# DavidSevic/gpu-nbody-simulation

Hardware: AMD Instinct MI355X
Metric: body-steps/sec (higher is better)
Workload: dtype f32

## Files before the change

### gpu-nbody-simulation_amd/csrc/bh_engine.hip

```cpp
#include "../../include/bhgpu.h"

#include <hip/hip_runtime.h>

#include <algorithm>
#include <cmath>
#include <cstdio>
#include <cstdlib>
#include <cstring>
#include <string>
#include <type_traits>
#include <vector>

#include "bh_tree.hpp"
#include "bh_walk_exact.hpp"
#include "bh_walk_f64.hpp"
#include "bh_diag.hpp"
#include "bh_direct.hpp"
#include "bh_field.hpp"
#include "bh_init.hpp"
#include "bh_let.hpp"
#include "bh_migrate.hpp"
#include "bh_walk_fast.h"

using namespace bh;
// ... 8 lines not shown
};
#endif

namespace {

thread_local std::string g_create_error;

struct DevBuf {
    void *p = nullptr;
    size_t bytes = 0;
};

}

struct bh_ctx {
    bh_config cfg{};
    int Dm = 0;
    enum class Mode { Exact, F64, Mixed, F32 };
    Mode mode = Mode::Exact;
    bool tree64() const { return mode == Mode::Exact || mode == Mode::F64; }
    bool state64() const { return mode != Mode::F32; }
    bool compat = true;
    bool exact_thresholds = false;
    int device = 0;
    hipStream_t stream = nullptr;
    bool own_stream = false;
    int64_t n = 0;
    bool uploaded = false, tree_valid = false;
    int64_t internal_cap = 0, node_cap = 0;
    int64_t bfs_max = 12288;
    int exact_bpw = 0;
    int walk_split = 0;
    bool walk_asm = true;
    int sort_bucket = 1;
    bool last_sort_bucket = false, last_sort_packed = false;
    int64_t samples_n = -1;
    uint64_t *splitters = nullptr;
    uint16_t *sort_dig = nullptr;
    int build_items = 0;
    bool hilbert = false;
    int partial_count = 0;
    double *bslots = nullptr;
    bool slots_valid = false;
    bool slots_dirty = true;

    void *pos = nullptr, *vel = nullptr, *mass = nullptr, *force = nullptr;
    void *pos2 = nullptr, *vel2 = nullptr, *mass2 = nullptr, *force2 = nullptr;
    uint32_t *orig = nullptr, *orig2 = nullptr;
    bool orig_identity = true;
    int reorder_every = 16;
    int64_t builds = 0;
    float2 *spos = nullptr;
    float4 *sstate = nullptr;
    float *smass = nullptr;
    uint64_t *keys[2] = {nullptr, nullptr};
    uint32_t *vals[2] = {nullptr, nullptr};
    uint64_t *keys_sorted = nullptr;
    uint32_t *perm = nullptr;
    uint32_t *radix_counts = nullptr, *bsum_sort = nullptr, *bsum_u32 = nullptr, *cnt = nullptr;
    uint64_t *coarse = nullptr;
    uint32_t *cell_first = nullptr;
    d3 *terms = nullptr, *bsum_d3 = nullptr;
    double *partial = nullptr, *box = nullptr;
    NodeD *gd = nullptr;
    LinkD *ld = nullptr;
    QuadF *qf = nullptr;
// ... 459 lines not shown
                               c->cfg.dt, w.integrate ? 1 : 0, c->ctr, w.slots, k.bpw, c->box);
        };
        dispatch([&](auto compat) {
            constexpr bool CP = decltype(compat)::value;
            if (!c->exact_thresholds) { if (w.stats) go(walk_exact_kernel<CP, true, false, false>); else go(walk_exact_kernel<CP, false, false, false>); }
            else if (w.stats) go(walk_exact_kernel<CP, true, true, false>);
            else if (k.use_asm) go(walk_exact_kernel<CP, false, true, true>);
            else go(walk_exact_kernel<CP, false, true, false>);
        }, c->compat);
        return BH_OK;
    });
}

int launch_walk_f32(bh_ctx *c, const WalkRange &w, const WalkChoice &k)
{
    WalkFastArgs a{};
    a.quads = c->qf; a.aux = c->aux; a.partial = w.partial; a.spos = c->spos; a.smass = c->smass; a.perm = c->perm;
    a.pos = (float2 *)c->pos; a.vel = (float2 *)c->vel;
    a.state64 = c->state64() ? 1 : 0;
    a.sstate = c->sstate;
    a.acc_out = (float2 *)c->force; a.ctr = c->ctr;
    a.lo = w.lo; a.hi = w.hi; a.G = (float)c->cfg.G; a.dt = (float)c->cfg.dt;
    a.integrate = w.integrate ? 1 : 0; a.to_sorted = w.to_sorted ? 1 : 0;
    a.n_trees = c->let_mode ? c->world : 0; a.self_rank = c->let_mode ? c->rank : -1;
    a.part = w.part; a.acc_part = c->acc_part;
    a.forest_base = c->forest_base; a.let_cap = c->let_cap;
    c->exp.walk_args(a);
    a.group_cost = (w.lo == 0 && w.hi == c->n) ? c->group_cost : nullptr;
    a.bucket_consts = c->walk_consts;
    a.slots = w.slots;
    a.body_counts = w.stats ? c->body_counts : nullptr;
    const bool lds = (c->cfg.flags & BH_FLAG_LDS_STACK) != 0;
    a.pair_limit = std::max(0, 116 - 3 * c->Dm);
    int split = (c->cfg.flags & BH_FLAG_WALK_NO_SPLIT) || c->cfg.n_threads > 0 ? 1 : c->walk_split;
    if (split <= 0) {
        const int64_t groups = (w.hi - w.lo + kWave - 1) / kWave;
        split = groups <= (c->let_mode ? 512 : 768) ? 8 : groups <= 3072 ? 4 : 1;
    }
    if (3 * c->Dm + 2 > kWave) split = 1;
    const int per_record = walk_fast_split_effective(a, lds, split) ? kWave : kBlock;
    if (w.partial) c->partial_count = (int)blocks_for(w.hi - w.lo, per_record);
    return each_pass(c, w, per_record, [&](int64_t plo, int64_t phi, unsigned) -> int {
        a.lo = plo; a.hi = phi; a.partial = w.partial ? w.partial + 4 * ((plo - w.lo) / per_record) : nullptr;
        BH_HIP(c, launch_walk_fast(a, lds, w.stats, split, k.use_asm, c->stream));
        return BH_OK;
    });
}

int enqueue_walk(bh_ctx *c, bool integrate, bool to_sorted, int part = 0)
{
    WalkRange w{};
    owned_range(c, &w.lo, &w.hi);
    if (w.hi <= w.lo) return BH_OK;
    w.integrate = integrate; w.to_sorted = to_sorted; w.part = part;
    w.stats = (c->cfg.flags & BH_FLAG_WALK_STATS) != 0;
    if (part != 2) c->walk_launches = 0;
    w.pass = c->cfg.n_threads > 0 ? ((int64_t)c->cfg.n_threads + kBlock - 1) / kBlock * kBlock : w.hi - w.lo;
    const bool full = integrate && !to_sorted && w.lo == 0 && w.hi == c->n;
    if (full && c->let_mode) w.partial = c->partial;
    const bool want_slots = full && part == 0 && !c->let_mode && !c->external_box && c->n >= 2;
    if (want_slots) { clean_slots(c); w.slots = c->bslots; }
    if (integrate) { c->slots_valid = want_slots; c->phi_current = false; }

    const WalkChoice k = choose_walk(c, w);
    if (w.stats && (k.kind == WalkKind::F64 || k.kind == WalkKind::F32)) {
        if (!c->body_counts) { int rc = dev_alloc(c, &c->body_counts, (size_t)std::max<int64_t>(c->cfg.capacity, 1)); if (rc) return rc; }
// ... 57 lines not shown
const char *bh_build_info(void) { return BHGPU_BUILD_INFO; }

const char *bh_last_error(const bh_ctx *ctx) { return ctx ? ctx->err.c_str() : g_create_error.c_str(); }

int bh_create(const bh_config *cfg, bh_ctx **out)
{
    if (!cfg || !out) return fail(nullptr, BH_ERR_ARG, "bh_create: null argument");
    *out = nullptr;
    if (cfg->capacity < 0 || cfg->capacity > 0x7fffffffLL - 8)
        return fail(nullptr, BH_ERR_ARG, "bh_create: capacity out of range");
    if (cfg->max_depth < 1 || cfg->max_depth > 32)
        return fail(nullptr, BH_ERR_ARG, "bh_create: max_depth must be 1..32");
    if (!(cfg->theta > 0.0)) return fail(nullptr, BH_ERR_ARG, "bh_create: theta must be > 0");
    if (cfg->precision != BH_PRECISION_F64_EXACT && cfg->precision != BH_PRECISION_F32 &&
        cfg->precision != BH_PRECISION_MIXED && cfg->precision != BH_PRECISION_F64)
        return fail(nullptr, BH_ERR_ARG, "bh_create: unknown precision");
    int ndev = 0;
    if (hipGetDeviceCount(&ndev) != hipSuccess || ndev <= 0)
        return fail(nullptr, BH_ERR_NO_DEVICE, "bh_create: no HIP device (libbhgpu has no CPU fallback)");
    if (cfg->device < 0 || cfg->device >= ndev)
        return fail(nullptr, BH_ERR_ARG, "bh_create: device ordinal out of range");

    bh_ctx *c = new bh_ctx();
    c->cfg = *cfg;
    c->Dm = cfg->max_depth - 1;
    c->mode = cfg->precision == BH_PRECISION_F64_EXACT ? Mode::Exact
            : cfg->precision == BH_PRECISION_F64       ? Mode::F64
            : cfg->precision == BH_PRECISION_MIXED     ? Mode::Mixed : Mode::F32;
    c->compat = cfg->reference_compat != 0;
    c->device = cfg->device;
    if (const char *e = std::getenv("BH_WALK_SPLIT")) c->walk_split = std::atoi(e);
    if (const char *e = std::getenv("BH_EXACT_BPW")) { const int b = std::atoi(e); c->exact_bpw = (b >= 1 && b <= kWave && (b & (b - 1)) == 0) ? b : 0; }
    if (const char *e = std::getenv("BH_WALK_ASM")) c->walk_asm = std::atoi(e) != 0;
    if (const char *e = std::getenv("BH_EXACT_BFS_MAX")) c->bfs_max = std::max(0, std::atoi(e));
    c->exact_thresholds = c->mode == Mode::Exact && c->walk_asm && !(cfg->flags & BH_FLAG_WALK_PORTABLE);
    if (const char *e = std::getenv("BH_SORT_PACK")) c->sort_pack = std::atoi(e) != 0;
    if (const char *e = std::getenv("BH_SORT_BUCKET")) c->sort_bucket = std::atoi(e);
    if (const char *e = std::getenv("BH_BUILD_ITEMS")) c->build_items = std::atoi(e);
    if (const char *e = std::getenv("BH_REORDER_EVERY")) c->reorder_every = std::max(0, std::atoi(e));
    c->hilbert = !c->tree64();
    if (const char *e = std::getenv("BH_HILBERT")) c->hilbert = !c->tree64() && std::atoi(e) != 0;
    auto bail = [&](int rc) { g_create_error = c->err; bh_destroy(c); return rc; };

    if (hipSetDevice(c->device) != hipSuccess) { c->err = "hipSetDevice failed"; return bail(BH_ERR_DEVICE); }
    if (hipStreamCreateWithFlags(&c->stream, hipStreamNonBlocking) != hipSuccess) {
        c->err = "hipStreamCreate failed"; return bail(BH_ERR_DEVICE);
    }
    c->own_stream = true;

    const int64_t cap = std::max<int64_t>(cfg->capacity, 1);
    c->node_cap = cfg->node_capacity > 0 ? cfg->node_capacity : 8 * cap + 1024;
    if (c->Dm < 15) {
        int64_t full = 0, wdt = 1;
        for (int l = 0; l <= c->Dm; ++l) { full += wdt; wdt *= 4; }
        c->node_cap = std::min(c->node_cap, std::max<int64_t>(full, 1));
    }
    c->internal_cap = (c->node_cap - 1) / 4;

    const size_t rs = c->state64() ? sizeof(double) : sizeof(float);
    int rc = 0;
    auto A = [&](auto **pp, size_t count) { if (!rc) rc = dev_alloc(c, pp, count); };
    { char *t; A(&t, cap * 2 * rs); c->pos = t; }
    { char *t; A(&t, cap * 2 * rs); c->vel = t; }
    { char *t; A(&t, cap * rs); c->mass = t; }
    { char *t; A(&t, cap * 2 * (c->tree64() ? sizeof(double) : sizeof(float))); c->force = t; }
    if (!c->tree64()) {
// ... 1217 lines not shown
```

### gpu-nbody-simulation_amd/csrc/bh_walk_fast.h

```cpp
#pragma once

#include <hip/hip_runtime.h>
#include <stdint.h>

namespace bh {

struct QuadF;
struct NodeAux;
struct TreeCounters;

struct WalkFastArgs {
    const QuadF *quads;
    const NodeAux *aux;
    const float2 *spos;
    const float *smass;
    const uint32_t *perm;
    float2 *pos, *vel;
    int32_t state64;
    float4 *sstate;
    float2 *acc_out;
    TreeCounters *ctr;
    double *partial;
    int64_t lo, hi;
    float G, dt;
    int integrate, to_sorted;
    uint32_t nblocks, pad0;
    const void *bucket_consts;
    uint32_t *group_cost;
    int32_t pair_limit;
    uint64_t *timeline;
    int32_t n_trees, self_rank;
    int32_t part;
    float2 *acc_part;
    int64_t forest_base, let_cap;
    double *slots;
    uint32_t *body_counts;
};

hipError_t launch_walk_fast(const WalkFastArgs &a, bool lds_stack, bool stats, int split, bool use_asm, hipStream_t st);
inline bool walk_fast_split_effective(const WalkFastArgs &a, bool lds_stack, int split)
{
    return split > 1 && !lds_stack && a.n_trees <= 56;
}

}
```

### gpu-nbody-simulation_amd/csrc/bh_walk_fast.hip

```cpp
#include "bh_prims.hpp"
#include "bh_nodes.hpp"
#include "bh_bounds.hpp"
#include "bh_walk_fast.h"
#include <cstdlib>

namespace bh {

#define BH_CONSTANT __attribute__((address_space(4)))

extern "C" __device__ int bh_writelane_i32(int value, int lane, int old) __asm("llvm.amdgcn.writelane.i32");

template <typename T>
__device__ __forceinline__ const T BH_CONSTANT *as_constant(const T *p)
{
#pragma clang diagnostic push
#pragma clang diagnostic ignored "-Wold-style-cast"
    return (const T BH_CONSTANT *)p;
#pragma clang diagnostic pop
}

typedef int32_t v16i __attribute__((ext_vector_type(16)));
typedef int32_t v4i __attribute__((ext_vector_type(4)));
typedef int32_t v2i __attribute__((ext_vector_type(2)));
struct QuadRegs { v16i g; v4i c; };
// ... 15 lines not shown
#define BH_LOOP_GUARD ""
#endif
#define BH_FORCE_MATH(MS, MASK)                                                                     \
    "v_mul_f32_e32 v26, " MS ", v25\n"                                                              \
    "v_mul_f32_e32 v26, v25, v26\n"                                                                 \
    "v_mul_f32_e32 v24, v25, v26\n"                                                                 \
    "v_fmac_f32_e32 v28, v24, v22\n"                                                                \
    "v_fmac_f32_e32 v29, v24, v23\n"                                                                \
    "s_mov_b64 exec, " MASK "\n"
#define BH_CHILD_HEAD(XY, MS, TS, MASK, SPAIR, TAG)                                                 \
    "s_cmp_eq_u32 " MS ", 0\n"                                                                      \
    "s_cbranch_scc1 Lnext" TAG "_%=\n"                                                              \
    "v_pk_add_f32 v[22:23], " XY ", v[20:21] neg_lo:[0,1] neg_hi:[0,1]\n"                           \
    "s_nop 0\n"                                                                                     \
    "v_mul_f32_e32 v24, v23, v23\n"                                                                 \
    "v_fmac_f32_e32 v24, v22, v22\n"                                                                \
    "v_cmpx_lt_f32_e32 vcc, " TS ", v24\n"                                                          \
    "v_rsq_f32_e32 v25, v24\n"                                                                      \
    "s_andn2_b64 " SPAIR ", " MASK ", vcc\n"                                                        \
    "s_cbranch_scc0 Lforce" TAG "_%=\n"
#define BH_CHILD_T(XY, MS, TS, CS, MASK, SPAIR, SLO, SHI, TAG, PUSHCHK)                             \
    BH_CHILD_HEAD(XY, MS, TS, MASK, SPAIR, TAG)                                                     \
    "s_cmp_eq_u32 " CS ", -1\n"                                                                     \
    "s_cbranch_scc1 Lforce" TAG "_%=\n"                                                             \
    PUSHCHK                                                                                         \
    "v_writelane_b32 v30, " CS ", m0\n"                                                             \
    "v_writelane_b32 v31, " SLO ", m0\n"                                                            \
    "v_writelane_b32 v32, " SHI ", m0\n"                                                            \
    "LpushBack" TAG "_%=:\n"                                                                        \
    "s_add_u32 m0, m0, 1\n"                                                                         \
    "Lforce" TAG "_%=:\n"                                                                           \
    BH_FORCE_MATH(MS, MASK)                                                                         \
    "Lnext" TAG "_%=:\n"
#define BH_CHILD_F(XY, MS, TS, CS, MASK, TAG, PUSHCHK)                                              \
    BH_CHILD_HEAD(XY, MS, TS, MASK, "s[68:69]", TAG)                                                \
    "s_cmp_gt_i32 " CS ", 0\n"                                                                      \
    "s_cbranch_scc1 Ltake" TAG "_%=\n"                                                              \
    "s_cmp_eq_u32 " CS ", -1\n"                                                                     \
    "s_cbranch_scc1 Lforce" TAG "_%=\n"                                                             \
    PUSHCHK                                                                                         \
    "v_writelane_b32 v30, " CS ", m0\n"                                                             \
    "v_writelane_b32 v31, s68, m0\n"                                                                \
    "v_writelane_b32 v32, s69, m0\n"                                                                \
    "LpushBack" TAG "_%=:\n"                                                                        \
    "s_add_u32 m0, m0, 1\n"                                                                         \
    "Lforce" TAG "_%=:\n"                                                                           \
    BH_FORCE_MATH(MS, MASK)                                                                         \
    "Lnext" TAG "_%=:\n"
#define BH_TAKE(MS, CS, MASK, NIDX, TAG, NEXT)                                                      \
    "Ltake" TAG "_%=:\n"                                                                            \
    "s_mov_b32 " NIDX ", " CS "\n"                                                                  \
    BH_FORCE_MATH(MS, MASK)                                                                         \
    "s_branch " NEXT "_%=\n"
#define BH_PUSHCHK(TAG) "s_bitcmp1_b32 m0, 6\n s_cbranch_scc1 LpushHi" TAG "_%=\n"
#define BH_NOCHK(TAG) ""
#define BH_PUSH_HI(CS, SLO, SHI, TAG)                                                               \
    "LpushHi" TAG "_%=:\n"                                                                          \
    "v_writelane_b32 v33, " CS ", m0\n"                                                             \
    "v_writelane_b32 v34, " SLO ", m0\n"                                                            \
    "v_writelane_b32 v35, " SHI ", m0\n"                                                            \
    "s_branch LpushBack" TAG "_%=\n"
#define BH_POP_FAST(IDX, LO, HI)                                                                    \
    "s_lshl_b64 exec, 1, m0\n"                                                                      \
    "v_readfirstlane_b32 " IDX ", v30\n v_readfirstlane_b32 " LO ", v31\n v_readfirstlane_b32 " HI ", v32\n"
#define BH_POP(IDX, LO, HI, TAG)                                                                    \
    "s_lshl_b64 exec, 1, m0\n"                                                                      \
    "s_bitcmp1_b32 m0, 6\n"                                                                         \
    "s_cbranch_scc1 LpopHi" TAG "_%=\n"                                                             \
    "v_readfirstlane_b32 " IDX ", v30\n v_readfirstlane_b32 " LO ", v31\n v_readfirstlane_b32 " HI ", v32\n" \
    "LpopBack" TAG "_%=:\n"
#define BH_POP_HI(IDX, LO, HI, TAG)                                                                 \
    "LpopHi" TAG "_%=:\n"                                                                           \
    "v_readfirstlane_b32 " IDX ", v33\n v_readfirstlane_b32 " LO ", v34\n v_readfirstlane_b32 " HI ", v35\n" \
    "s_branch LpopBack" TAG "_%=\n"
#define BH_ITERATION(SFX, POPA, POPB, CHK)                                                              \
                   \
    "s_cmp_gt_i32 s72, -1\n"                                                                        \
    "s_cbranch_scc1 LAn" SFX "_%=\n"                                                                \
    "s_sub_u32 m0, m0, 1\n"                                  \
    "s_cbranch_scc1 LAe" SFX "_%=\n"                                                                \
    POPA                                                                                            \
    "s_cmp_lt_i32 s68, 0\n"                                                                         \
    "s_cbranch_scc1 Lspecial_%=\n"                                                                  \
// ... 2 lines not shown
    "s_mov_b32 m0, 0\n"                                                                             \
    "s_cmp_lt_i32 s70, 0\n"                                                                         \
    "s_cbranch_scc1 Ldone_%=\n"                                                                     \
    "s_mov_b32 s68, s70\n"                                                                          \
    "s_mov_b64 s[44:45], s[46:47]\n"                                                                \
    "s_mov_b32 s70, -1\n"                                                                           \
    "s_branch LAr" SFX "_%=\n"                                                                      \
    "LAn" SFX "_%=:\n"                                                                              \
    "s_mov_b32 s68, s72\n"                                   \
    "LAr" SFX "_%=:\n"                                    \
    "s_mul_i32 s69, s68, 0x50\n"                                                                    \
    "s_load_dwordx16 s[24:39], %[quads], s69\n"                                                     \
    "s_load_dwordx4 s[40:43], %[quads], s69 offset:0x40\n"                                          \
        \
    "s_cmp_gt_i32 s70, -1\n"                                                                        \
    "s_cbranch_scc1 LBn" SFX "_%=\n"                                                                \
    "s_mov_b64 s[46:47], 0\n"                                             \
    "s_cmp_eq_u32 m0, 0\n"                                                                          \
    "s_cbranch_scc1 LW" SFX "_%=\n"                                                                 \
    "s_cmp_gt_u32 m0, %[plim]\n"                                                                    \
    "s_cbranch_scc1 LW" SFX "_%=\n"                                                                 \
    "s_sub_u32 m0, m0, 1\n"                                                                         \
    POPB                                                                                            \
    "s_cmp_lt_i32 s70, 0\n"                                                                         \
    "s_cbranch_scc1 Lunpop" SFX "_%=\n"                                                             \
    "LBn" SFX "_%=:\n"                                                                              \
    "s_mul_i32 s71, s70, 0x50\n"                                                                    \
    "s_load_dwordx16 s[48:63], %[quads], s71\n"                                                     \
    "s_load_dwordx4 s[64:67], %[quads], s71 offset:0x40\n"                                          \
    "LW" SFX "_%=:\n"                                                                               \
    "s_mov_b64 exec, s[44:45]\n"                                                                    \
    "s_waitcnt lgkmcnt(0)\n"                                                                                    \
    "s_setprio 0\n"                                                                                 \
                                                         \
    BH_CHILD_F("s[24:25]", "s32", "s36", "s40", "s[44:45]", SFX "A0f", CHK(SFX "A0f"))              \
    BH_CHILD_F("s[26:27]", "s33", "s37", "s41", "s[44:45]", SFX "A1f", CHK(SFX "A1f"))              \
    BH_CHILD_F("s[28:29]", "s34", "s38", "s42", "s[44:45]", SFX "A2f", CHK(SFX "A2f"))              \
    BH_CHILD_F("s[30:31]", "s35", "s39", "s43", "s[44:45]", SFX "A3f", CHK(SFX "A3f"))              \
    "s_mov_b32 s72, -1\n"                                                  \
    "s_branch LphB" SFX "_%=\n"                                                                     \
      \
    "LA1t" SFX "_%=:\n"                                                                             \
    BH_CHILD_T("s[26:27]", "s33", "s37", "s41", "s[44:45]", "s[70:71]", "s70", "s71", SFX "A1t", CHK(SFX "A1t")) \
    "LA2t" SFX "_%=:\n"                                                                             \
    BH_CHILD_T("s[28:29]", "s34", "s38", "s42", "s[44:45]", "s[70:71]", "s70", "s71", SFX "A2t", CHK(SFX "A2t")) \
    "LA3t" SFX "_%=:\n"                                                                             \
    BH_CHILD_T("s[30:31]", "s35", "s39", "s43", "s[44:45]", "s[70:71]", "s70", "s71", SFX "A3t", CHK(SFX "A3t")) \
    "LAet" SFX "_%=:\n"                                                                             \
    "s_mov_b64 s[44:45], s[68:69]\n"                      \
    "s_mov_b32 s70, -1\n"                                 \
    "LphB" SFX "_%=:\n"                                                                             \
    "s_cmp_eq_u64 s[46:47], 0\n"                                                                    \
    "s_cbranch_scc1 Lloop_%=\n"                                           \
    "s_mov_b64 exec, s[46:47]\n"                                                                    \
    "s_cmp_gt_u32 m0, %[plim]\n"                          \
    "s_cbranch_scc1 LBover" SFX "_%=\n"                                                             \
    BH_CHILD_F("s[48:49]", "s56", "s60", "s64", "s[46:47]", SFX "B0f", CHK(SFX "B0f"))              \
    BH_CHILD_F("s[50:51]", "s57", "s61", "s65", "s[46:47]", SFX "B1f", CHK(SFX "B1f"))              \
    BH_CHILD_F("s[52:53]", "s58", "s62", "s66", "s[46:47]", SFX "B2f", CHK(SFX "B2f"))              \
    BH_CHILD_F("s[54:55]", "s59", "s63", "s67", "s[46:47]", SFX "B3f", CHK(SFX "B3f"))              \
    "s_mov_b32 s70, -1\n"                                                                           \
    "s_branch Lloop_%=\n"                                                                           \
    "LB0t" SFX "_%=:\n"                                                                             \
    BH_CHILD_T("s[48:49]", "s56", "s60", "s64", "s[46:47]", "s[24:25]", "s24", "s25", SFX "B0t", CHK(SFX "B0t")) \
    "LB1t" SFX "_%=:\n"                                                                             \
    BH_CHILD_T("s[50:51]", "s57", "s61", "s65", "s[46:47]", "s[24:25]", "s24", "s25", SFX "B1t", CHK(SFX "B1t")) \
    "LB2t" SFX "_%=:\n"                                                                             \
    BH_CHILD_T("s[52:53]", "s58", "s62", "s66", "s[46:47]", "s[24:25]", "s24", "s25", SFX "B2t", CHK(SFX "B2t")) \
    "LB3t" SFX "_%=:\n"                                                                             \
    BH_CHILD_T("s[54:55]", "s59", "s63", "s67", "s[46:47]", "s[24:25]", "s24", "s25", SFX "B3t", CHK(SFX "B3t")) \
    "LBet" SFX "_%=:\n"                                                                             \
    "s_mov_b64 s[46:47], s[68:69]\n"                      \
    "s_branch Lloop_%=\n"                                                                           \
    "Lunpop" SFX "_%=:\n"                                 \
    "s_add_u32 m0, m0, 1\n"                                                                         \
    "s_mov_b32 s70, -1\n"                                                                           \
    "s_mov_b64 s[46:47], 0\n"                                                                       \
    "s_branch LW" SFX "_%=\n"                                                                       \
    "LBover" SFX "_%=:\n"                                   \
    "s_mov_b32 s70, -1\n"                                                                           \
    "s_branch LB0t" SFX "_%=\n"                                                                     \
    BH_TAKE("s32", "s40", "s[44:45]", "s72", SFX "A0f", "LA1t" SFX)                                 \
    BH_TAKE("s33", "s41", "s[44:45]", "s72", SFX "A1f", "LA2t" SFX)                                 \
    BH_TAKE("s34", "s42", "s[44:45]", "s72", SFX "A2f", "LA3t" SFX)                                 \
    BH_TAKE("s35", "s43", "s[44:45]", "s72", SFX "A3f", "LAet" SFX)                                 \
    BH_TAKE("s56", "s64", "s[46:47]", "s70", SFX "B0f", "LB1t" SFX)                                 \
    BH_TAKE("s57", "s65", "s[46:47]", "s70", SFX "B1f", "LB2t" SFX)                                 \
    BH_TAKE("s58", "s66", "s[46:47]", "s70", SFX "B2f", "LB3t" SFX)                                 \
    BH_TAKE("s59", "s67", "s[46:47]", "s70", SFX "B3f", "LBet" SFX)
#define BH_HI_STUBS(SFX)                                                                            \
    BH_PUSH_HI("s40", "s68", "s69", SFX "A0f") BH_PUSH_HI("s41", "s68", "s69", SFX "A1f")          \
    BH_PUSH_HI("s42", "s68", "s69", SFX "A2f") BH_PUSH_HI("s43", "s68", "s69", SFX "A3f")          \
    BH_PUSH_HI("s41", "s70", "s71", SFX "A1t") BH_PUSH_HI("s42", "s70", "s71", SFX "A2t")          \
    BH_PUSH_HI("s43", "s70", "s71", SFX "A3t")                                                     \
    BH_PUSH_HI("s64", "s68", "s69", SFX "B0f") BH_PUSH_HI("s65", "s68", "s69", SFX "B1f")          \
    BH_PUSH_HI("s66", "s68", "s69", SFX "B2f") BH_PUSH_HI("s67", "s68", "s69", SFX "B3f")          \
    BH_PUSH_HI("s64", "s24", "s25", SFX "B0t") BH_PUSH_HI("s65", "s24", "s25", SFX "B1t")          \
    BH_PUSH_HI("s66", "s24", "s25", SFX "B2t") BH_PUSH_HI("s67", "s24", "s25", SFX "B3t")

#define BH_TREE_LOOP(LIMITCHK) \
     \
    "Lloop_%=:\n" \
    "s_add_u32 %[cost], %[cost], 1\n" \
    BH_LOOP_GUARD LIMITCHK \
    "s_setprio 2\n" \
    "s_cmp_gt_u32 m0, 56\n" \
    "s_cbranch_scc1 LloopChk_%=\n" \
    BH_ITERATION("F", BH_POP_FAST("s68", "s44", "s45"), BH_POP_FAST("s70", "s46", "s47"), BH_NOCHK) \
    "LloopChk_%=:\n"  \
    BH_ITERATION("C", BH_POP("s68", "s44", "s45", "A"), BH_POP("s70", "s46", "s47", "B"), BH_PUSHCHK) \
    BH_HI_STUBS("C") \
    BH_POP_HI("s68", "s44", "s45", "A") \
    BH_POP_HI("s70", "s46", "s47", "B") \
     \
     \
     \
    "Lspecial_%=:\n" \
    "s_cmp_eq_u32 s68, -1\n" \
    "s_cbranch_scc1 Lloop_%=\n" \
    "s_load_dwordx8 s[56:63], %[consts], 0x0\n"  \
    "s_sub_i32 s68, -2, s68\n" \
    "s_lshl_b32 s69, s68, 3\n" \
    "s_mov_b64 exec, s[44:45]\n" \
    "s_waitcnt lgkmcnt(0)\n" \
    "s_load_dwordx2 s[48:49], s[56:57], s69\n"  \
    "s_waitcnt lgkmcnt(0)\n" \
    "s_cmp_lt_i32 s49, 1\n" \
    "s_cbranch_scc1 Lloop_%=\n" \
    "s_add_u32 s49, s48, s49\n" \
// ... 172 lines not shown
    constexpr int FCAP = SPLIT > 1 ? kSplitFrontier : 1;
    __shared__ int32_t fr_base[2][FCAP], fr_lo[2][FCAP], fr_hi[2][FCAP];
    __shared__ int32_t f_cnt[SPLIT > 1 ? SPLIT : 1];
    __shared__ float2 f_red[SPLIT > 1 ? SPLIT : 1][SPLIT > 1 ? kWave : 1];

    if (a.ctr->overflow) return;
#ifdef BHGPU_EXPERIMENTS
    const uint64_t dbg_t0 = a.timeline ? __builtin_amdgcn_s_memrealtime() : 0;
    const uint64_t dbg_c0 = a.timeline ? __builtin_amdgcn_s_memtime() : 0;
#endif
    const uint32_t lb = blockIdx.x;
    if (lb >= a.nblocks) return;
    const int lane = lane_id(), w = wave_id();
    const int64_t s = SPLIT > 1 ? a.lo + (int64_t)lb * kWave + lane : a.lo + (int64_t)lb * kBlock + threadIdx.x;
    bool valid = s < a.hi;
    const float2 p = valid ? a.spos[s] : float2{0.f, 0.f};
    asm volatile("" ::"v"(p.x), "v"(p.y));
    float ax = 0.f, ay = 0.f;
    if (a.part == 2 && valid && (SPLIT == 1 || w == 0)) { const float2 t = a.acc_part[s]; ax = t.x; ay = t.y; }
    asm volatile("" : "+v"(ax), "+v"(ay));
    unsigned long long n_vis = 0, n_int = 0, n_wave = 0, n_quad = 0;
    uint32_t my_int = 0;
    uint32_t cost = 0;

    const QuadF BH_CONSTANT *quads = as_constant(a.quads);
    const NodeAux BH_CONSTANT *aux = as_constant(a.aux);
    const float2 BH_CONSTANT *cpos = as_constant(a.spos);
    const float BH_CONSTANT *cmass = as_constant(a.smass);

    int32_t v_base = 0, v_lo = 0, v_hi = 0;
    int32_t v_base2 = 0, v_lo2 = 0, v_hi2 = 0;
    int sp = 0;

    bool h_free = false;
    int32_t h_idx = -1;
    uint64_t h_mask = 0;

    auto eval = [&](const float cx, const float cy, const int32_t mbits, const float thr, const int32_t child,
                    const uint64_t mask) {
        if (mbits == 0) return;
        const float m = __int_as_float(mbits);
        const float dx = cx - p.x, dy = cy - p.y;
        const float d2 = fmaf(dx, dx, dy * dy);
        const uint64_t farm = __ballot(d2 > thr);
        const uint64_t accm = mask & farm;
        const float ri = __builtin_amdgcn_rsqf(d2);
        const float wgt = __builtin_amdgcn_inverse_ballot_w64(accm) ? m * ri * ri * ri : 0.f;
        ax = fmaf(wgt, dx, ax);
        ay = fmaf(wgt, dy, ay);
        if (STATS) { n_vis += __popcll(mask); ++n_wave; n_int += __popcll(accm); my_int += (uint32_t)((accm >> lane) & 1ull); }
        if (child != -1) {
            const uint64_t open = mask & ~farm;
            if (open != 0 && h_free && child > 0) {
                h_idx = child; h_mask = open; h_free = false;
            } else if (open != 0) {
                if (LDS_STACK) {
                    if (lane == 0) { s_base[w][sp] = child; s_mask[w][sp] = open; }
                } else if (sp < kWave) {
                    v_base = bh_writelane_i32(child, sp, v_base);
                    v_lo = bh_writelane_i32((int32_t)(uint32_t)open, sp, v_lo);
                    v_hi = bh_writelane_i32((int32_t)(uint32_t)(open >> 32), sp, v_hi);
                } else {
                    v_base2 = bh_writelane_i32(child, sp - kWave, v_base2);
                    v_lo2 = bh_writelane_i32((int32_t)(uint32_t)open, sp - kWave, v_lo2);
                    v_hi2 = bh_writelane_i32((int32_t)(uint32_t)(open >> 32), sp - kWave, v_hi2);
                }
                ++sp;
            }
        }
    };

    auto eval_quad = [&](const QuadRegs &q, const uint64_t mask) {
        if (STATS) ++n_quad;
        eval(__int_as_float(q.g[0]), __int_as_float(q.g[1]), q.g[8], __int_as_float(q.g[12]), q.c[0], mask);
        eval(__int_as_float(q.g[2]), __int_as_float(q.g[3]), q.g[9], __int_as_float(q.g[13]), q.c[1], mask);
        eval(__int_as_float(q.g[4]), __int_as_float(q.g[5]), q.g[10], __int_as_float(q.g[14]), q.c[2], mask);
        eval(__int_as_float(q.g[6]), __int_as_float(q.g[7]), q.g[11], __int_as_float(q.g[15]), q.c[3], mask);
    };

    auto bucket = [&](const int32_t node, const uint64_t mask) {
#pragma clang diagnostic push
#pragma clang diagnostic ignored "-Wold-style-cast"
        const v2i rng = *(const v2i BH_CONSTANT *)(aux + node);
        for (int32_t j = rng[0]; j < rng[0] + rng[1]; ++j) {
            const v2i ob = *(const v2i BH_CONSTANT *)(cpos + j);
            const float om = *(const float BH_CONSTANT *)(cmass + j);
#pragma clang diagnostic pop
            const float dx = __int_as_float(ob[0]) - p.x, dy = __int_as_float(ob[1]) - p.y;
// ... 133 lines not shown
            cur ^= 1;
            F = produced;
        }
        f_red[w][lane] = float2{ax, ay};
        __syncthreads();
        if (w == 0) {
#pragma unroll
            for (int k = 1; k < SPLIT; ++k) { ax += f_red[k][lane].x; ay += f_red[k][lane].y; }
        }
        valid = valid && (w == 0);
    } else {
        const uint64_t everyone = __ballot(valid);
        const int32_t t_first = (a.part == 2) ? 0 : -1, t_end = (a.part == 1) ? 0 : a.n_trees;
        for (int32_t t = t_first; t < t_end; ++t) {
            if (t >= 0 && t == a.self_rank) continue;
            int32_t base = (t < 0) ? 0 : (int32_t)(a.forest_base + (int64_t)t * a.let_cap);
            if (ASM) {
                cost += walk_tree_asm(quads, as_constant(a.bucket_consts), base, everyone, a.pair_limit, p.x, p.y, ax, ay);
                continue;
            }
            {
                int32_t na = -1, nb = -1;
                uint64_t nam = 0, nbm = 0;
                bool first = true;
                for (;;) {
                    int32_t bA, bB = -1;
                    uint64_t mA, mB = 0;
                    ++cost;
                    if (first) { bA = base; mA = everyone; first = false; }
                    else {
                        if (na >= 0) { bA = na; mA = nam; }
                        else if (sp > 0) {
                            pop_raw(bA, mA);
                            if (bA < 0) {
                                if (bA <= -2) bucket(-bA - 2, mA);
                                continue;
                            }
                        } else if (nb >= 0) { bA = nb; mA = nbm; nb = -1; }
                        else break;
                        if (nb >= 0) { bB = nb; mB = nbm; }
                        else if (sp > 0 && sp <= a.pair_limit) {
                            pop_raw(bB, mB);
                            if (bB < 0) { ++sp; bB = -1; }
                        }
                    }
                    const QuadRegs A = load_quad(quads + bA);
                    QuadRegs B = A;
                    if (bB >= 0) B = load_quad(quads + bB);
                    h_free = true; h_idx = -1;
                    eval_quad(A, mA);
                    na = h_idx; nam = h_mask;
                    nb = -1;
                    if (bB >= 0) {
                        h_free = sp <= a.pair_limit; h_idx = -1;
                        eval_quad(B, mB);
                        nb = h_idx; nbm = h_mask;
                    }
                    h_free = false;
                }
            }
        }
    }

    const WalkFastArgs BH_CONSTANT *ka;
    {
#pragma clang diagnostic push
#pragma clang diagnostic ignored "-Wold-style-cast"
        ka = (const WalkFastArgs BH_CONSTANT *)__builtin_amdgcn_kernarg_segment_ptr();
#pragma clang diagnostic pop
    }
    asm volatile("" : "+s"(ka));
    const WalkFastArgs BH_CONSTANT &e = *ka;
    float2 np = p;
    double2 np64{0.0, 0.0};
    if (e.part == 1) {
        if (valid) e.acc_part[s] = float2{ax, ay};
    } else if (valid) {
        const float gx = e.G * ax, gy = e.G * ay;
        const uint32_t body = e.perm[s];
        if (e.acc_out) e.acc_out[body] = float2{gx, gy};
        if (e.integrate && e.state64) {
            double2 *pos64 = reinterpret_cast<double2 *>(e.pos), *vel64 = reinterpret_cast<double2 *>(e.vel);
            double2 v = vel64[body];
            const double2 q = pos64[body];
            v.x = fma((double)gx, (double)e.dt, v.x);
            v.y = fma((double)gy, (double)e.dt, v.y);
            np64 = double2{fma(v.x, (double)e.dt, q.x), fma(v.y, (double)e.dt, q.y)};
            vel64[body] = v;
            pos64[body] = np64;
        } else if (e.integrate) {
            float2 v = e.vel[body];
// ... 41 lines not shown
    }
    if (STATS && e.body_counts && s < e.hi && my_int) atomicAdd(&e.body_counts[e.perm[s]], my_int);
    if (STATS && lane == 0) {
        atomicAdd(&e.ctr->visits, n_vis);
        atomicAdd(&e.ctr->interactions, n_int);
        atomicAdd(&e.ctr->wave_nodes, n_wave);
        atomicAdd(&e.ctr->wave_quads, n_quad);
    }
}

template <bool L, bool S, int SPLIT = 1, bool ASM = false>
static hipError_t launch(WalkFastArgs a, hipStream_t st)
{
    const int64_t cnt = a.hi - a.lo;
    if (cnt <= 0) return hipSuccess;
    constexpr int per_group = SPLIT > 1 ? kWave : kBlock;
    a.nblocks = (uint32_t)((cnt + per_group - 1) / per_group);
    hipLaunchKernelGGL((walk_fast_kernel<L, S, SPLIT, ASM>), dim3(a.nblocks), dim3(SPLIT > 1 ? kWave * SPLIT : kBlock), 0, st, a);
    return hipGetLastError();
}

template <bool S, bool ASM = false>
static hipError_t launch_split(const WalkFastArgs &a, int split, hipStream_t st)
{
    switch (split) {
    case 2: return launch<false, S, 2, ASM>(a, st);
    case 4: return launch<false, S, 4, ASM>(a, st);
    default: return launch<false, S, 8, ASM>(a, st);
    }
}

hipError_t launch_walk_fast(const WalkFastArgs &a, bool lds_stack, bool stats, int split, bool use_asm, hipStream_t st)
{
    if (use_asm && !lds_stack && !stats && !walk_fast_split_effective(a, lds_stack, split))
        return launch<false, false, 1, true>(a, st);
    if (walk_fast_split_effective(a, lds_stack, split))
        return stats ? launch_split<true>(a, split, st)
                     : (use_asm ? launch_split<false, true>(a, split, st) : launch_split<false>(a, split, st));
    if (lds_stack) return stats ? launch<true, true>(a, st) : launch<true, false>(a, st);
    return stats ? launch<false, true>(a, st) : launch<false, false>(a, st);
}

}
```

Baseline: 2.376 billion.

## Hand off a second opened child to the B slot in the tree walk

Extends the Barnes-Hut walk's register handoff so that when evaluating quad A, a second opened child can go straight into the B slot for the next iteration instead of being pushed onto and popped from the stack. It covers both the C++ walk loop and the inline-asm walker, adding new label paths (A1g..A3g, A2u/A3u) that check the pair limit before taking. The aim is fewer stack push/pop operations and more paired quad evaluations per iteration. The cost is more complex assembly control flow and extra scalar register use. A BH_WALK_HANDOFF env knob plus experiment-only histogram instrumentation are also added.

Measured after the change: 2.373 billion (median of 2 runs). About the same (-0.1%).

```diff
diff --git a/gpu-nbody-simulation_amd/csrc/bh_engine.hip b/gpu-nbody-simulation_amd/csrc/bh_engine.hip
--- a/gpu-nbody-simulation_amd/csrc/bh_engine.hip
+++ b/gpu-nbody-simulation_amd/csrc/bh_engine.hip
@@ -64,6 +64,7 @@
     int exact_bpw = 0;
     int walk_split = 0;
     bool walk_asm = true;
+    int walk_handoff = 2;
     int sort_bucket = 1;
     bool last_sort_bucket = false, last_sort_packed = false;
     int64_t samples_n = -1;
@@ -589,6 +590,7 @@
     a.body_counts = w.stats ? c->body_counts : nullptr;
     const bool lds = (c->cfg.flags & BH_FLAG_LDS_STACK) != 0;
     a.pair_limit = std::max(0, 116 - 3 * c->Dm);
+    a.handoff = c->walk_handoff;
     int split = (c->cfg.flags & BH_FLAG_WALK_NO_SPLIT) || c->cfg.n_threads > 0 ? 1 : c->walk_split;
     if (split <= 0) {
         const int64_t groups = (w.hi - w.lo + kWave - 1) / kWave;
@@ -712,6 +714,7 @@
     if (const char *e = std::getenv("BH_WALK_SPLIT")) c->walk_split = std::atoi(e);
     if (const char *e = std::getenv("BH_EXACT_BPW")) { const int b = std::atoi(e); c->exact_bpw = (b >= 1 && b <= kWave && (b & (b - 1)) == 0) ? b : 0; }
     if (const char *e = std::getenv("BH_WALK_ASM")) c->walk_asm = std::atoi(e) != 0;
+    if (const char *e = std::getenv("BH_WALK_HANDOFF")) c->walk_handoff = std::min(2, std::max(0, std::atoi(e)));
     if (const char *e = std::getenv("BH_EXACT_BFS_MAX")) c->bfs_max = std::max(0, std::atoi(e));
     c->exact_thresholds = c->mode == Mode::Exact && c->walk_asm && !(cfg->flags & BH_FLAG_WALK_PORTABLE);
     if (const char *e = std::getenv("BH_SORT_PACK")) c->sort_pack = std::atoi(e) != 0;
diff --git a/gpu-nbody-simulation_amd/csrc/bh_walk_fast.h b/gpu-nbody-simulation_amd/csrc/bh_walk_fast.h
--- a/gpu-nbody-simulation_amd/csrc/bh_walk_fast.h
+++ b/gpu-nbody-simulation_amd/csrc/bh_walk_fast.h
@@ -24,10 +24,12 @@
     int64_t lo, hi;
     float G, dt;
     int integrate, to_sorted;
-    uint32_t nblocks, pad0;
+    uint32_t nblocks;
+    int32_t handoff;
     const void *bucket_consts;
     uint32_t *group_cost;
     int32_t pair_limit;
+    uint64_t *handoff_hist;
     uint64_t *timeline;
     int32_t n_trees, self_rank;
     int32_t part;
diff --git a/gpu-nbody-simulation_amd/csrc/bh_walk_fast.hip b/gpu-nbody-simulation_amd/csrc/bh_walk_fast.hip
--- a/gpu-nbody-simulation_amd/csrc/bh_walk_fast.hip
+++ b/gpu-nbody-simulation_amd/csrc/bh_walk_fast.hip
@@ -71,16 +71,17 @@
     "Lforce" TAG "_%=:\n"                                                                           \
     BH_FORCE_MATH(MS, MASK)                                                                         \
     "Lnext" TAG "_%=:\n"
-#define BH_CHILD_F(XY, MS, TS, CS, MASK, TAG, PUSHCHK)                                              \
-    BH_CHILD_HEAD(XY, MS, TS, MASK, "s[68:69]", TAG)                                                \
+#define BH_CHILD_F(XY, MS, TS, CS, MASK, SPAIR, SLO, SHI, TAG, PUSHCHK)                             \
+    BH_CHILD_HEAD(XY, MS, TS, MASK, SPAIR, TAG)                                                     \
     "s_cmp_gt_i32 " CS ", 0\n"                                                                      \
     "s_cbranch_scc1 Ltake" TAG "_%=\n"                                                              \
     "s_cmp_eq_u32 " CS ", -1\n"                                                                     \
     "s_cbranch_scc1 Lforce" TAG "_%=\n"                                                             \
+    "Lpush" TAG "_%=:\n"                                                                            \
     PUSHCHK                                                                                         \
     "v_writelane_b32 v30, " CS ", m0\n"                                                             \
-    "v_writelane_b32 v31, s68, m0\n"                                                                \
-    "v_writelane_b32 v32, s69, m0\n"                                                                \
+    "v_writelane_b32 v31, " SLO ", m0\n"                                                            \
+    "v_writelane_b32 v32, " SHI ", m0\n"                                                            \
     "LpushBack" TAG "_%=:\n"                                                                        \
     "s_add_u32 m0, m0, 1\n"                                                                         \
     "Lforce" TAG "_%=:\n"                                                                           \
@@ -88,6 +89,14 @@
     "Lnext" TAG "_%=:\n"
 #define BH_TAKE(MS, CS, MASK, NIDX, TAG, NEXT)                                                      \
     "Ltake" TAG "_%=:\n"                                                                            \
+    "s_mov_b32 " NIDX ", " CS "\n"                                                                  \
+    BH_FORCE_MATH(MS, MASK)                                                                         \
+    "s_branch " NEXT "_%=\n"
+#define BH_TAKE_LIM(MS, CS, MASK, NIDX, TAG, NEXT)                                                  \
+    "Ltake" TAG "_%=:\n"                                                                            \
+    "s_add_u32 vcc_lo, m0, 3\n"                                                                     \
+    "s_cmp_gt_u32 vcc_lo, %[plim]\n"                                                                \
+    "s_cbranch_scc1 Lpush" TAG "_%=\n"                                                              \
     "s_mov_b32 " NIDX ", " CS "\n"                                                                  \
     BH_FORCE_MATH(MS, MASK)                                                                         \
     "s_branch " NEXT "_%=\n"
@@ -156,20 +165,21 @@
     "s_mov_b64 exec, s[44:45]\n"                                                                    \
     "s_waitcnt lgkmcnt(0)\n"                                                                                    \
     "s_setprio 0\n"                                                                                 \
-                                                         \
-    BH_CHILD_F("s[24:25]", "s32", "s36", "s40", "s[44:45]", SFX "A0f", CHK(SFX "A0f"))              \
-    BH_CHILD_F("s[26:27]", "s33", "s37", "s41", "s[44:45]", SFX "A1f", CHK(SFX "A1f"))              \
-    BH_CHILD_F("s[28:29]", "s34", "s38", "s42", "s[44:45]", SFX "A2f", CHK(SFX "A2f"))              \
-    BH_CHILD_F("s[30:31]", "s35", "s39", "s43", "s[44:45]", SFX "A3f", CHK(SFX "A3f"))              \
+     \
+    BH_CHILD_F("s[24:25]", "s32", "s36", "s40", "s[44:45]", "s[68:69]", "s68", "s69", SFX "A0f", CHK(SFX "A0f")) \
+    BH_CHILD_F("s[26:27]", "s33", "s37", "s41", "s[44:45]", "s[68:69]", "s68", "s69", SFX "A1f", CHK(SFX "A1f")) \
+    BH_CHILD_F("s[28:29]", "s34", "s38", "s42", "s[44:45]", "s[68:69]", "s68", "s69", SFX "A2f", CHK(SFX "A2f")) \
+    BH_CHILD_F("s[30:31]", "s35", "s39", "s43", "s[44:45]", "s[68:69]", "s68", "s69", SFX "A3f", CHK(SFX "A3f")) \
     "s_mov_b32 s72, -1\n"                                                  \
     "s_branch LphB" SFX "_%=\n"                                                                     \
-      \
-    "LA1t" SFX "_%=:\n"                                                                             \
-    BH_CHILD_T("s[26:27]", "s33", "s37", "s41", "s[44:45]", "s[70:71]", "s70", "s71", SFX "A1t", CHK(SFX "A1t")) \
-    "LA2t" SFX "_%=:\n"                                                                             \
-    BH_CHILD_T("s[28:29]", "s34", "s38", "s42", "s[44:45]", "s[70:71]", "s70", "s71", SFX "A2t", CHK(SFX "A2t")) \
-    "LA3t" SFX "_%=:\n"                                                                             \
-    BH_CHILD_T("s[30:31]", "s35", "s39", "s43", "s[44:45]", "s[70:71]", "s70", "s71", SFX "A3t", CHK(SFX "A3t")) \
+     \
+                                                                  \
+    "LA1g" SFX "_%=:\n"                                                                             \
+    BH_CHILD_F("s[26:27]", "s33", "s37", "s41", "s[44:45]", "s[70:71]", "s70", "s71", SFX "A1g", CHK(SFX "A1g")) \
+    "LA2g" SFX "_%=:\n"                                                                             \
+    BH_CHILD_F("s[28:29]", "s34", "s38", "s42", "s[44:45]", "s[70:71]", "s70", "s71", SFX "A2g", CHK(SFX "A2g")) \
+    "LA3g" SFX "_%=:\n"                                                                             \
+    BH_CHILD_F("s[30:31]", "s35", "s39", "s43", "s[44:45]", "s[70:71]", "s70", "s71", SFX "A3g", CHK(SFX "A3g")) \
     "LAet" SFX "_%=:\n"                                                                             \
     "s_mov_b64 s[44:45], s[68:69]\n"                      \
     "s_mov_b32 s70, -1\n"                                 \
@@ -179,12 +189,14 @@
     "s_mov_b64 exec, s[46:47]\n"                                                                    \
     "s_cmp_gt_u32 m0, %[plim]\n"                          \
     "s_cbranch_scc1 LBover" SFX "_%=\n"                                                             \
-    BH_CHILD_F("s[48:49]", "s56", "s60", "s64", "s[46:47]", SFX "B0f", CHK(SFX "B0f"))              \
-    BH_CHILD_F("s[50:51]", "s57", "s61", "s65", "s[46:47]", SFX "B1f", CHK(SFX "B1f"))              \
-    BH_CHILD_F("s[52:53]", "s58", "s62", "s66", "s[46:47]", SFX "B2f", CHK(SFX "B2f"))              \
-    BH_CHILD_F("s[54:55]", "s59", "s63", "s67", "s[46:47]", SFX "B3f", CHK(SFX "B3f"))              \
+       \
+    BH_CHILD_F("s[48:49]", "s56", "s60", "s64", "s[46:47]", "s[70:71]", "s70", "s71", SFX "B0f", CHK(SFX "B0f")) \
+    BH_CHILD_F("s[50:51]", "s57", "s61", "s65", "s[46:47]", "s[70:71]", "s70", "s71", SFX "B1f", CHK(SFX "B1f")) \
+    BH_CHILD_F("s[52:53]", "s58", "s62", "s66", "s[46:47]", "s[70:71]", "s70", "s71", SFX "B2f", CHK(SFX "B2f")) \
+    BH_CHILD_F("s[54:55]", "s59", "s63", "s67", "s[46:47]", "s[70:71]", "s70", "s71", SFX "B3f", CHK(SFX "B3f")) \
     "s_mov_b32 s70, -1\n"                                                                           \
     "s_branch Lloop_%=\n"                                                                           \
+     \
     "LB0t" SFX "_%=:\n"                                                                             \
     BH_CHILD_T("s[48:49]", "s56", "s60", "s64", "s[46:47]", "s[24:25]", "s24", "s25", SFX "B0t", CHK(SFX "B0t")) \
     "LB1t" SFX "_%=:\n"                                                                             \
@@ -194,31 +206,48 @@
     "LB3t" SFX "_%=:\n"                                                                             \
     BH_CHILD_T("s[54:55]", "s59", "s63", "s67", "s[46:47]", "s[24:25]", "s24", "s25", SFX "B3t", CHK(SFX "B3t")) \
     "LBet" SFX "_%=:\n"                                                                             \
-    "s_mov_b64 s[46:47], s[68:69]\n"                      \
+    "s_mov_b64 s[46:47], s[70:71]\n"                      \
+    "s_mov_b32 s70, s40\n"                                                                          \
     "s_branch Lloop_%=\n"                                                                           \
     "Lunpop" SFX "_%=:\n"                                 \
     "s_add_u32 m0, m0, 1\n"                                                                         \
     "s_mov_b32 s70, -1\n"                                                                           \
     "s_mov_b64 s[46:47], 0\n"                                                                       \
     "s_branch LW" SFX "_%=\n"                                                                       \
-    "LBover" SFX "_%=:\n"                                   \
-    "s_mov_b32 s70, -1\n"                                                                           \
+    "LBover" SFX "_%=:\n"                                                                           \
+    "s_mov_b32 s40, -1\n"                                                                           \
     "s_branch LB0t" SFX "_%=\n"                                                                     \
-    BH_TAKE("s32", "s40", "s[44:45]", "s72", SFX "A0f", "LA1t" SFX)                                 \
-    BH_TAKE("s33", "s41", "s[44:45]", "s72", SFX "A1f", "LA2t" SFX)                                 \
-    BH_TAKE("s34", "s42", "s[44:45]", "s72", SFX "A2f", "LA3t" SFX)                                 \
+     \
+                                                     \
+    "LA2u" SFX "_%=:\n"                                                                             \
+    BH_CHILD_T("s[28:29]", "s34", "s38", "s42", "s[44:45]", "s[24:25]", "s24", "s25", SFX "A2u", CHK(SFX "A2u")) \
+    "LA3u" SFX "_%=:\n"                                                                             \
+    BH_CHILD_T("s[30:31]", "s35", "s39", "s43", "s[44:45]", "s[24:25]", "s24", "s25", SFX "A3u", CHK(SFX "A3u")) \
+    "LAeu" SFX "_%=:\n"                                                                             \
+    "s_mov_b64 s[44:45], s[68:69]\n"                                                                \
+    "s_cmp_eq_u64 s[46:47], 0\n"                                                                    \
+    "s_cbranch_scc1 LBet" SFX "_%=\n"                                                               \
+    "s_mov_b64 exec, s[46:47]\n"                                                                    \
+    "s_branch LB0t" SFX "_%=\n"                                                                     \
+    BH_TAKE("s32", "s40", "s[44:45]", "s72", SFX "A0f", "LA1g" SFX)                                 \
+    BH_TAKE("s33", "s41", "s[44:45]", "s72", SFX "A1f", "LA2g" SFX)                                 \
+    BH_TAKE("s34", "s42", "s[44:45]", "s72", SFX "A2f", "LA3g" SFX)                                 \
     BH_TAKE("s35", "s43", "s[44:45]", "s72", SFX "A3f", "LAet" SFX)                                 \
-    BH_TAKE("s56", "s64", "s[46:47]", "s70", SFX "B0f", "LB1t" SFX)                                 \
-    BH_TAKE("s57", "s65", "s[46:47]", "s70", SFX "B1f", "LB2t" SFX)                                 \
-    BH_TAKE("s58", "s66", "s[46:47]", "s70", SFX "B2f", "LB3t" SFX)                                 \
-    BH_TAKE("s59", "s67", "s[46:47]", "s70", SFX "B3f", "LBet" SFX)
+    BH_TAKE_LIM("s33", "s41", "s[44:45]", "s40", SFX "A1g", "LA2u" SFX)                             \
+    BH_TAKE_LIM("s34", "s42", "s[44:45]", "s40", SFX "A2g", "LA3u" SFX)                             \
+    BH_TAKE_LIM("s35", "s43", "s[44:45]", "s40", SFX "A3g", "LAeu" SFX)                             \
+    BH_TAKE("s56", "s64", "s[46:47]", "s40", SFX "B0f", "LB1t" SFX)                                 \
+    BH_TAKE("s57", "s65", "s[46:47]", "s40", SFX "B1f", "LB2t" SFX)                                 \
+    BH_TAKE("s58", "s66", "s[46:47]", "s40", SFX "B2f", "LB3t" SFX)                                 \
+    BH_TAKE("s59", "s67", "s[46:47]", "s40", SFX "B3f", "LBet" SFX)
 #define BH_HI_STUBS(SFX)                                                                            \
     BH_PUSH_HI("s40", "s68", "s69", SFX "A0f") BH_PUSH_HI("s41", "s68", "s69", SFX "A1f")          \
     BH_PUSH_HI("s42", "s68", "s69", SFX "A2f") BH_PUSH_HI("s43", "s68", "s69", SFX "A3f")          \
-    BH_PUSH_HI("s41", "s70", "s71", SFX "A1t") BH_PUSH_HI("s42", "s70", "s71", SFX "A2t")          \
-    BH_PUSH_HI("s43", "s70", "s71", SFX "A3t")                                                     \
-    BH_PUSH_HI("s64", "s68", "s69", SFX "B0f") BH_PUSH_HI("s65", "s68", "s69", SFX "B1f")          \
-    BH_PUSH_HI("s66", "s68", "s69", SFX "B2f") BH_PUSH_HI("s67", "s68", "s69", SFX "B3f")          \
+    BH_PUSH_HI("s41", "s70", "s71", SFX "A1g") BH_PUSH_HI("s42", "s70", "s71", SFX "A2g")          \
+    BH_PUSH_HI("s43", "s70", "s71", SFX "A3g")                                                     \
+    BH_PUSH_HI("s42", "s24", "s25", SFX "A2u") BH_PUSH_HI("s43", "s24", "s25", SFX "A3u")          \
+    BH_PUSH_HI("s64", "s70", "s71", SFX "B0f") BH_PUSH_HI("s65", "s70", "s71", SFX "B1f")          \
+    BH_PUSH_HI("s66", "s70", "s71", SFX "B2f") BH_PUSH_HI("s67", "s70", "s71", SFX "B3f")          \
     BH_PUSH_HI("s64", "s24", "s25", SFX "B0t") BH_PUSH_HI("s65", "s24", "s25", SFX "B1t")          \
     BH_PUSH_HI("s66", "s24", "s25", SFX "B2t") BH_PUSH_HI("s67", "s24", "s25", SFX "B3t")
 
@@ -457,9 +486,18 @@
     int32_t v_base2 = 0, v_lo2 = 0, v_hi2 = 0;
     int sp = 0;
 
-    bool h_free = false;
-    int32_t h_idx = -1;
-    uint64_t h_mask = 0;
+    bool h_free = false, g_free = false;
+    int32_t h_idx = -1, g_idx = -1;
+    uint64_t h_mask = 0, g_mask = 0;
+#ifdef BHGPU_EXPERIMENTS
+    int q_open = 0;
+    auto hist = [&](int k) { if (STATS && a.handoff_hist && lane == 0) atomicAdd(a.handoff_hist + k, 1ull); };
+#define BH_HIST(k) hist(k)
+#define BH_HIST_OPEN() (++q_open)
+#else
+#define BH_HIST(k) ((void)0)
+#define BH_HIST_OPEN() ((void)0)
+#endif
 
     auto eval = [&](const float cx, const float cy, const int32_t mbits, const float thr, const int32_t child,
                     const uint64_t mask) {
@@ -476,9 +514,13 @@
         if (STATS) { n_vis += __popcll(mask); ++n_wave; n_int += __popcll(accm); my_int += (uint32_t)((accm >> lane) & 1ull); }
         if (child != -1) {
             const uint64_t open = mask & ~farm;
+            if (open != 0 && child > 0) BH_HIST_OPEN();
             if (open != 0 && h_free && child > 0) {
                 h_idx = child; h_mask = open; h_free = false;
+            } else if (open != 0 && g_free && child > 0 && sp + 3 <= a.pair_limit) {
+                g_idx = child; g_mask = open; g_free = false;
             } else if (open != 0) {
+                BH_HIST(child > 0 ? 55 : 56);
                 if (LDS_STACK) {
                     if (lane == 0) { s_base[w][sp] = child; s_mask[w][sp] = open; }
                 } else if (sp < kWave) {
@@ -678,6 +720,7 @@
                         if (na >= 0) { bA = na; mA = nam; }
                         else if (sp > 0) {
                             pop_raw(bA, mA);
+                            BH_HIST(57);
                             if (bA < 0) {
                                 if (bA <= -2) bucket(-bA - 2, mA);
                                 continue;
@@ -688,21 +731,39 @@
                         else if (sp > 0 && sp <= a.pair_limit) {
                             pop_raw(bB, mB);
                             if (bB < 0) { ++sp; bB = -1; }
+                            else BH_HIST(57);
                         }
                     }
                     const QuadRegs A = load_quad(quads + bA);
                     QuadRegs B = A;
                     if (bB >= 0) B = load_quad(quads + bB);
-                    h_free = true; h_idx = -1;
+                    h_free = a.handoff >= 1; h_idx = -1;
+                    g_free = a.handoff >= 2; g_idx = -1;
                     eval_quad(A, mA);
                     na = h_idx; nam = h_mask;
-                    nb = -1;
+                    nb = g_idx; nbm = g_mask;
+                    g_free = false;
+#ifdef BHGPU_EXPERIMENTS
+                    const int oA = q_open;
+                    q_open = 0;
+                    BH_HIST(oA);
+                    if (na >= 0) BH_HIST(58);
+                    if (nb >= 0) BH_HIST(59);
+#endif
                     if (bB >= 0) {
-                        h_free = sp <= a.pair_limit; h_idx = -1;
+                        h_free = a.handoff >= 1 && nb < 0 && sp <= a.pair_limit; h_idx = -1;
                         eval_quad(B, mB);
-                        nb = h_idx; nbm = h_mask;
+                        if (nb < 0) { nb = h_idx; nbm = h_mask; }
+#ifdef BHGPU_EXPERIMENTS
+                        BH_HIST(q_open);
+                        if (h_idx >= 0) BH_HIST(60);
+#endif
                     }
                     h_free = false;
+#ifdef BHGPU_EXPERIMENTS
+                    BH_HIST(5 + (bB >= 0 ? 25 : 0) + 5 * oA + q_open);
+                    q_open = 0;
+#endif
                 }
             }
         }
@@ -810,7 +871,7 @@
 
 hipError_t launch_walk_fast(const WalkFastArgs &a, bool lds_stack, bool stats, int split, bool use_asm, hipStream_t st)
 {
-    if (use_asm && !lds_stack && !stats && !walk_fast_split_effective(a, lds_stack, split))
+    if (use_asm && a.handoff >= 2 && !lds_stack && !stats && !walk_fast_split_effective(a, lds_stack, split))
         return launch<false, false, 1, true>(a, st);
     if (walk_fast_split_effective(a, lds_stack, split))
         return stats ? launch_split<true>(a, split, st)
```
